# hammershock/SFM-Python

Hardware: AMD Instinct MI355X
Metric: BA iterations/sec (higher is better)
Workload: dtype f64

## Files before the change

### include/sfmba.h

```cpp
#ifndef SFMBA_H
#define SFMBA_H

#include <stdint.h>

#ifdef __cplusplus
extern "C" {
#endif

typedef struct sfmba_handle sfmba_handle;

typedef struct sfmba_options {
    double  ftol;
    double  xtol;
    double  gtol;
    int64_t max_nfev;
    int32_t verbose;
    int32_t max_iter;
    double  pcg_tol;
    int32_t pcg_max_iter;
    int32_t pcg_check_every;
    double  reg_min;
    int32_t profile;
    int32_t reserved;
    double  pcg_tol_max;
// ... 160 lines not shown
void sfmba_default_pose_options(sfmba_pose_options* opt);
int  sfmba_recover_pose(sfmba_handle* h, int64_t n_edges, const int64_t* edge_ptr, const double* pts1, const double* pts2,
                        const uint8_t* pair_use , const double* E, const double* K,
                        const sfmba_pose_options* opt, double* R, double* t, uint8_t* front_mask, double* X, double* angle_deg,
                        int32_t* edge_front, int32_t* edge_front_all, double* edge_sum_err, int32_t* edge_status,
                        int64_t* n_ok, double* kernel_us);

int  sfmba_set_descriptors(sfmba_handle* h, int64_t n_images, const int64_t* img_ptr ,
                           const void* desc , int32_t dtype ,
                           int32_t dim , int32_t* form_out);
typedef struct sfmba_match_options {
    double  ratio;
    int32_t form;
    int32_t profile;
} sfmba_match_options;
void sfmba_default_match_options(sfmba_match_options* opt);
int  sfmba_match_descriptors(sfmba_handle* h, int64_t n_edges, const int32_t* edges ,
                             const sfmba_match_options* opt, int64_t* query_ptr , int32_t* idx ,
                             double* dist_sq , uint8_t* good , int32_t* edge_good, int32_t* edge_status,
                             int64_t* n_ok, double* kernel_us);

int  sfmba_solve(sfmba_handle* h, double* x_inout, const sfmba_options* opt, sfmba_result* out);
int  sfmba_solve_from(sfmba_handle* h, const double* x0, double* x_out, const sfmba_options* opt, sfmba_result* out);
int  sfmba_get_fun_grad(sfmba_handle* h, double* fun_out, double* grad_out);

int  sfmba_time_kernel(sfmba_handle* h, const double* x, int32_t which, int32_t reps, double* avg_us);
int  sfmba_normal_blocks(sfmba_handle* h, const double* x, double* U, double* V, double* gc,
                         double* gp);
int  sfmba_schur_matvec(sfmba_handle* h, const double* x, const double* dc, const double* dp,
                        const double* v, double* y);

int  sfmba_step_products(sfmba_handle* h, const double* x, const double* sg, const double* dc, const double* dp_diag,
                         double* t1_out, double* g11_out, double* dp_out, double* sums_out, double* g_out, double* si_out);

int  sfmba_rhs_precond(sfmba_handle* h, const double* x, const double* dc, const double* dp, double* rhs_out,
                       double* sd_out, double* minv_out);

int  sfmba_dense_schur(sfmba_handle* h, const double* x, const double* dc, const double* dp, const double* rhs,
                       double* S_out, double* sol_out);

int  sfmba_tr2d_solve(const double* B3, const double* g2, double Delta, double* p2);
int  sfmba_debug_option(sfmba_handle* h, const char* name, int64_t value);

#ifdef __cplusplus
}
#endif
// ... 2 lines not shown
```

### sfm-python_amd/csrc/sfmba.hip

```cpp
#include "../../include/sfmba.h"

#include <hip/hip_runtime.h>
#include <hip/hip_ext.h>
#include <rccl/rccl.h>
#include <dlfcn.h>

#include <algorithm>
#include <atomic>
#include <chrono>
#include <cmath>
#include <cstdarg>
#include <cstdio>
#include <cstdlib>
#include <cstring>
#include <condition_variable>
#include <functional>
#include <initializer_list>
#include <mutex>
#include <numeric>
#include <string>
#include <thread>
#include <vector>

#include "problem_tables.hpp"
#include "ba_kernels.hpp"
#include "consumer_kernels.hpp"
#include "match_kernels.hpp"
#include "tr2d.hpp"

using namespace sfmba;

namespace {

constexpr size_t kLdsBytes = 160 * 1024;
constexpr size_t kLdsDynMax = kLdsBytes - 2048;
constexpr int kScalSlots = 32;
constexpr int kPartRows = 2048;
constexpr int kCostSlot = 0, kG11Slot = 1, kTailSlot = 2, kQ1Slot = 8;
constexpr int kMaxSlot = 12, kRegSlot = 13, kGhPrevSlot = 14, kEtaSlot = 15, kCamSlot = 16;
constexpr int kStepSlot = 25, kSkipSlot = 30, kRadiusSlot = 31;
constexpr int kPinCtrl = 40;
constexpr int kPinP2pErr = 62;
constexpr int kPointSlot[9] = {12, 8, 9, 10, 11, 4, 5, 6, 7};

struct DevBuf {
    void* p = nullptr;
    size_t bytes = 0;
// ... 23 lines not shown

struct DevView {
    void* p = nullptr;
    template <class T> T* as() const { return static_cast<T*>(p); }
};

struct PinnedBuf {
    void* p = nullptr;
    size_t bytes = 0;
    ~PinnedBuf() { if (p) (void)hipHostFree(p); }
    hipError_t ensure(size_t n, size_t keep) {
        if (n <= bytes && p) return hipSuccess;
        void* q = nullptr;
        const size_t cap = n + n / 2 + 64;
        hipError_t e = hipHostMalloc(&q, cap, hipHostMallocDefault);
        if (e != hipSuccess) return e;
        if (p && keep) memcpy(q, p, std::min(keep, bytes));
        if (p) (void)hipHostFree(p);
        p = q; bytes = cap;
        return hipSuccess;
    }
    template <class T> T* as() const { return static_cast<T*>(p); }
};

struct RcclApi {
    void* lib = nullptr;
    ncclResult_t (*GetUniqueId)(ncclUniqueId*) = nullptr;
    ncclResult_t (*CommInitRank)(ncclComm_t*, int, ncclUniqueId, int) = nullptr;
    ncclResult_t (*AllReduce)(const void*, void*, size_t, ncclDataType_t, ncclRedOp_t, ncclComm_t, hipStream_t) = nullptr;
    ncclResult_t (*CommDestroy)(ncclComm_t) = nullptr;
    const char* (*GetErrorString)(ncclResult_t) = nullptr;
};
RcclApi* rccl_api() {
    static RcclApi api;
    static bool tried = false;
    if (!tried) {
        tried = true;
        void* lib = dlopen("librccl.so.1", RTLD_NOW | RTLD_GLOBAL);
        if (!lib) lib = dlopen("librccl.so", RTLD_NOW | RTLD_GLOBAL);
        if (!lib) lib = dlopen("/opt/rocm/lib/librccl.so.1", RTLD_NOW | RTLD_GLOBAL);
        if (lib) {
            api.GetUniqueId = (decltype(api.GetUniqueId))dlsym(lib, "ncclGetUniqueId");
            api.CommInitRank = (decltype(api.CommInitRank))dlsym(lib, "ncclCommInitRank");
            api.AllReduce = (decltype(api.AllReduce))dlsym(lib, "ncclAllReduce");
            api.CommDestroy = (decltype(api.CommDestroy))dlsym(lib, "ncclCommDestroy");
            api.GetErrorString = (decltype(api.GetErrorString))dlsym(lib, "ncclGetErrorString");
// ... 8 lines not shown
    X(pcg_fused, -1)       \
    X(tab_lds, -1)         \
    X(vec_lds, -1)         \
    X(sweep_rc, -1)        \
    X(dense, -1)           \
    X(precond, -1)         \
    X(pcg_local, -1)       \
    X(xcd_chunks, -1)      \
    X(rhsrec, -1)          \
    X(cost_rider, -1)      \
    X(packed_upload, -1)   \
    X(jfree, -1)           \
    X(rc_consumers, -1)    \
    X(cm_device, -1)       \
    X(pcg_inline, -1)      \
    X(xcd_cam, -1)         \
    X(pcg_skip_last, -1)   \
    X(pcg_mixed_b, -1)     \
    X(pcg_mixed, -1)       \
    X(pcg_split, -1)       \
    X(spec_scale, -1)      \
    X(start_handoff, -1)   \
    X(early_download, -1)  \
    X(cam_chunk, 0)        \
    X(pcg_guess_bias, 0)   \
    X(trace_pcg, 0) X(trace_stalls, 0) X(trace_timing, 0)    \
    X(wait_deadline_s, 120)  \
    X(p2p_delay_ms, 0)     \
    X(p2p_timeout_ms, 0)
struct Debug {
#define X(name, init) int name = init;
    SFMBA_DEBUG_OPTIONS(X)
#undef X
};
const struct { const char* name; int Debug::*member; } kDebugOptions[] = {
#define X(name, init) {#name, &Debug::name},
    SFMBA_DEBUG_OPTIONS(X)
#undef X
};

struct Forms {
    bool packed_upload = false;
    bool cm_device = false;
    int64_t cam_chunk_len = 4096;
    bool lds_tab = true, lds_vec = true;
    bool sweep_rc = false;
// ... 93 lines not shown
        double* camdata[kP2pMaxRanks] = {};
        unsigned* words = nullptr;
        int64_t calls = 0;
        bool first_in_solve = true;
        int shared_device = 1;
        bool any_multi = false;
    } p2p;
    double* h_scal = nullptr;
    struct Stage { PinnedBuf uv, ci, pi, perm, ptr, uvf, tables, ci16, uv16; } stage;
    DevBuf ci16_dev, uv16_dev;
    struct Prev { bool valid = false; bool f32 = false; bool packed = false; int64_t N = 0, P = 0; } prev;
    ProblemTables tb;
    HostPool pool;
    int64_t obs_reused = 0, obs_uploaded = 0;
    double* mbox = nullptr;
    double* mbox_dev = nullptr;
    unsigned long long mbox_seq = 0;
    Mailbox post{};
    double* h_x = nullptr;
    size_t h_x_doubles = 0;
    hipStream_t copy_stream = nullptr;
    hipEvent_t ev_written = nullptr, ev_copied[2] = {nullptr, nullptr};
    bool result_in_flight = false;
    PinnedBuf mirror[2];
    unsigned long long mirror_tag[2] = {0, 0}, copy_count = 0, x_tag = 0;
    bool mirror_on = false;
    const double* skip = nullptr;
    double pcg_tol = 0.0; int pcg_cap = 0;
    bool pcg_b_owed = false;
    bool pcg_a_owed = false;
    DevBuf pcg_part;
    int pcg_hint = 0;
    std::vector<int> pcg_hist;
    int64_t hist_C = 0, hist_P = 0, hist_N = 0;
    unsigned long long hist_sig = 0;
    unsigned long long problem_gen = 0;
    bool solved = false;
    bool transport_dropped = false;
    std::vector<const void*> lds_ready;
    int last_pcg_iters = 0;

    double *x = nullptr, *x_new = nullptr;
    double *tab = nullptr, *tab_new = nullptr;
    double *rec = nullptr, *rec_new = nullptr;
    double *g_cur = nullptr, *si_cur = nullptr, *sg_cur = nullptr;
    double *g_new = nullptr, *si_new = nullptr, *sg_new = nullptr;
// ... 704 lines not shown
    CHK(exchange(h, h->scal() + kQ1Slot, 4, 0));
    CHK(exchange(h, h->scal() + kMaxSlot, 1, 1));
    return 0;
}

int fetch_scalars(sfmba_handle* h) {
    const Mailbox mb{h->mbox_dev, h->scal(), nullptr, ++h->mbox_seq, p2p_error_word(h)};
    hipLaunchKernelGGL(k_post, dim3(1), dim3(64), 0, h->stream, mb);
    LAUNCHED(h);
    CHK(wait_mailbox(h, h->mbox_seq));
    memcpy(h->h_scal, h->mbox, sizeof(double) * kScalSlots);
    return 0;
}

int ensure_h_x(sfmba_handle* h) {
    const size_t need = (size_t)std::max<int64_t>(h->n, 2 * h->N);
    if (h->h_x && h->h_x_doubles >= need) return 0;
    if (h->h_x) { (void)hipHostFree(h->h_x); h->h_x = nullptr; h->h_x_doubles = 0; }
    HIPCHK(h, hipHostMalloc((void**)&h->h_x, sizeof(double) * need, hipHostMallocDefault));
    h->h_x_doubles = need;
    return 0;
}

template <class Fn>
void staging_copy(sfmba_handle* h, void* dst, const void* src, size_t bytes, Fn chunk_done) {
    const int parts = (int)std::min<size_t>(4, bytes >> 19);
    if (parts <= 1) { memcpy(dst, src, bytes); chunk_done(0, (size_t)0, bytes); return; }
    const size_t per = ((bytes + parts - 1) / parts + 63) & ~(size_t)63;
    std::atomic<int> done[8];
    for (auto& d : done) d.store(0, std::memory_order_relaxed);
    h->pool.run(parts, [&](int t) {
        const size_t b = std::min(bytes, (size_t)t * per), e = std::min(bytes, b + per);
        if (e > b) memcpy(static_cast<char*>(dst) + b, static_cast<const char*>(src) + b, e - b);
        if (t != 0) { done[t].store(1, std::memory_order_release); return; }
        chunk_done(0, b, e - b);
        for (int k = 1; k < parts; ++k) {
            while (done[k].load(std::memory_order_acquire) == 0) { }
            const size_t bk = std::min(bytes, (size_t)k * per), ek = std::min(bytes, bk + per);
            chunk_done(k, bk, ek - bk);
        }
    });
}
void staging_copy(sfmba_handle* h, void* dst, const void* src, size_t bytes) {
    staging_copy(h, dst, src, bytes, [](int, size_t, size_t) {});
}

int upload_x(sfmba_handle* h, const double* x_host, double* dst = nullptr) {
    CHK(ensure_h_x(h));
    if (h->forms.mixed && !dst) {
        const double* pts = x_host + 6 * h->C;
        const int64_t stride = std::max<int64_t>(1, h->P / 1024);
        double sx = 0.0, sy = 0.0, sz = 0.0;
        int64_t cnt = 0;
        for (int64_t q = 0; q < h->P; q += stride, ++cnt) { sx += pts[3 * q]; sy += pts[3 * q + 1]; sz += pts[3 * q + 2]; }
        h->origin = Origin{sx / (double)cnt, sy / (double)cnt, sz / (double)cnt};
        if (!std::isfinite(h->origin.x + h->origin.y + h->origin.z)) h->origin = Origin{0.0, 0.0, 0.0};
    }
    HIPCHK(h, hipStreamSynchronize(h->stream));
    if (h->result_in_flight && h->copy_stream) HIPCHK(h, hipStreamSynchronize(h->copy_stream));
    h->result_in_flight = false;
    const double t0 = now_s();
    hipError_t err = hipSuccess;
    staging_copy(h, h->h_x, x_host, sizeof(double) * h->n, [&](int, size_t off, size_t bytes) {
        if (bytes == 0 || err != hipSuccess) return;
        err = hipMemcpyAsync(reinterpret_cast<char*>(dst ? dst : h->x) + off, reinterpret_cast<const char*>(h->h_x) + off, bytes,
                             hipMemcpyHostToDevice, h->stream);
    });
    HIPCHK(h, err);
    if (h->dbg.trace_timing) fprintf(stderr, "sfmba: upload_x  staging copy + enqueue %.1f us\n", 1e6 * (now_s() - t0));
    return 0;
}

int download_residuals(sfmba_handle* h, double* r_out) {
    CHK(ensure_h_x(h));
    HIPCHK(h, hipStreamSynchronize(h->stream));
    const size_t bytes = (h->f32 ? sizeof(float) : sizeof(double)) * 2 * (size_t)h->N;
    HIPCHK(h, hipMemcpyAsync(h->h_x, h->r.p, bytes, hipMemcpyDeviceToHost, h->stream));
    CHK(wait_stream(h));
    if (!h->f32 && !h->permuted) { memcpy(r_out, h->h_x, bytes); return 0; }
    const float* sf = reinterpret_cast<const float*>(h->h_x);
    for (int64_t k = 0; k < h->N; ++k) {
        const int64_t d = h->permuted ? h->tb.order[k] : k;
        r_out[2 * d] = h->f32 ? (double)sf[2 * k] : h->h_x[2 * k];
        r_out[2 * d + 1] = h->f32 ? (double)sf[2 * k + 1] : h->h_x[2 * k + 1];
    }
    return 0;
// ... 176 lines not shown
    o->reg_min = 1e-6; o->profile = 0; o->reserved = 0; o->pcg_tol_max = 0.1;
}

int sfmba_create(sfmba_handle** out, int device_id) {
    if (!out) return -1;
    *out = nullptr;
    int ndev = 0;
    hipError_t e = hipGetDeviceCount(&ndev);
    if (e != hipSuccess || ndev <= 0) return -3;
    if (device_id < 0 || device_id >= ndev) return -1;
    auto* h = new sfmba_handle();
    h->device = device_id;
    if (hipSetDevice(device_id) != hipSuccess) { delete h; return -3; }
    hipDeviceProp_t prop;
    if (hipGetDeviceProperties(&prop, device_id) == hipSuccess) h->n_cu = prop.multiProcessorCount;
    if (hipStreamCreateWithFlags(&h->stream, hipStreamNonBlocking) != hipSuccess) { delete h; return -3; }
    h->own_stream = true;
    if (hipHostMalloc((void**)&h->h_scal, sizeof(double) * 64, hipHostMallocDefault) != hipSuccess ||
        hipHostMalloc((void**)&h->mbox, sizeof(double) * 64, hipHostMallocCoherent | hipHostMallocMapped) != hipSuccess ||
        hipHostGetDevicePointer((void**)&h->mbox_dev, h->mbox, 0) != hipSuccess) {
        (void)hipStreamDestroy(h->stream); delete h; return -4;
    }
    memset(h->mbox, 0, sizeof(double) * 64);
    {
        int prio_low = 0, prio_high = 0;
        if (hipDeviceGetStreamPriorityRange(&prio_low, &prio_high) != hipSuccess) prio_low = 0;
        if (hipStreamCreateWithPriority(&h->copy_stream, hipStreamNonBlocking, prio_low) != hipSuccess) h->copy_stream = nullptr;
    }
    if (h->copy_stream &&
        (hipEventCreateWithFlags(&h->ev_written, hipEventDisableTiming) != hipSuccess ||
         hipEventCreateWithFlags(&h->ev_copied[0], hipEventDisableTiming) != hipSuccess ||
         hipEventCreateWithFlags(&h->ev_copied[1], hipEventDisableTiming) != hipSuccess)) {
        (void)hipStreamDestroy(h->copy_stream);
        h->copy_stream = nullptr;
    }
    *out = h;
    return 0;
}

void sfmba_destroy(sfmba_handle* h) {
    if (!h) return;
    (void)hipSetDevice(h->device);
    if (h->stream) (void)hipStreamSynchronize(h->stream);
    if (h->comm) { if (RcclApi* api = rccl_api()) (void)api->CommDestroy(h->comm); h->comm = nullptr; }
    p2p_release(h);
    if (h->copy_stream) { (void)hipStreamSynchronize(h->copy_stream); (void)hipStreamDestroy(h->copy_stream); }
    if (h->ev_written) (void)hipEventDestroy(h->ev_written);
    for (auto& ev : h->ev_copied) if (ev) (void)hipEventDestroy(ev);
    if (h->own_stream && h->stream) (void)hipStreamDestroy(h->stream);
    if (h->h_scal) (void)hipHostFree(h->h_scal);
    if (h->mbox) (void)hipHostFree(h->mbox);
    if (h->h_x) (void)hipHostFree(h->h_x);
    delete h;
}

const char* sfmba_last_error(const sfmba_handle* h) { return h ? h->err.c_str() : "null handle"; }

int sfmba_set_stream(sfmba_handle* h, void* hip_stream) {
    CHK(enter(h));
    if (h->stream) HIPCHK(h, hipStreamSynchronize(h->stream));
    if (h->own_stream && h->stream) (void)hipStreamDestroy(h->stream);
    h->stream = static_cast<hipStream_t>(hip_stream);
    h->own_stream = false;
    return 0;
}

int sfmba_set_print(sfmba_handle* h, sfmba_print_fn fn, void* ctx) {
    CHK(enter(h));
    h->print_fn = fn;
    h->print_ctx = ctx;
    return 0;
}

int sfmba_debug_option(sfmba_handle* h, const char* name, int64_t value) {
    CHK(enter(h));
// ... 1843 lines not shown
    struct EventList : std::vector<std::pair<hipEvent_t, hipEvent_t>> {
        ~EventList() { for (auto& pr : *this) { (void)hipEventDestroy(pr.first); (void)hipEventDestroy(pr.second); } }
    } evs;
    int np_cost = 0;
    int np_tail = 0;
    double cost = 0.0, Delta = -1.0;
    unsigned long long start_seq = 0;
    int64_t nfev = 1, njev = 1, iteration = 0, pcg_total = 0, pcg_breakdowns = 0;
    int status = -1;
    double step_norm = 0.0, actual_reduction = 0.0, g_norm = 0.0, reg_term = 0.0, cost_new = 0.0;
    bool have_red = false;
    int pcg_guess = h->pcg_hint;
    bool guess_exact = false;
    bool hist_same = false;
    unsigned long long sig = 0;
    std::vector<int> pcg_hist_new;
    int pcg_enqueued = 0;
    bool missed = false;
    PcgCtrl hc{};
    bool nb_valid = true;
    Mailbox trial_post{};
    bool trial_post_pending = false;
    bool result_sent = false;
    double t_begin = 0.0, t_dev0 = 0.0, t_sent0 = 0.0, t_sent1 = 0.0;

    int run(const double* x_start, double* x_out);
    int start(const double* x_start), start_values();
    void recall_pcg_record(const double* x_start);
    int linear_phase(), tail();
    int device_trial();
    void record_pcg_count();
    int step_loop(), accept_or_reject(), terminate();
    int deliver(double* x_out);
    int eval_jac(const double* x, double* tab, bool table_ready, bool finish = true);
    int enqueue_trial(const double* coef_dev, double c1, double c2), handoff(bool with_ctrl);
    int fetch() {
        CHK(wait_mailbox(h, h->mbox_seq));
        memcpy(h->h_scal, h->mbox, sizeof(double) * kScalSlots);
        return 0;
    }
    double qsum(int q) const { return hs[kPointSlot[q]] + hs[kCamSlot + q]; }
    int guess_launches() const { return pcg_guess + (f.pcg_fused ? 1 : 0) + (guess_exact ? 0 : 1); }
};

int Solve::eval_jac(const double* x, double* tab, bool table_ready, bool finish) {
    if (!table_ready) CHK(launch_cam_table(h, x, tab, h->rec, f.quick_start));
// ... 268 lines not shown
        if (term != 0) { status = term; break; }
        Delta = Delta_new;
    }
    have_red = true;
    return 0;
}

int Solve::accept_or_reject() {
    if (!(actual_reduction > 0.0)) {
        step_norm = 0.0;
        actual_reduction = 0.0;
        return 0;
    }
    std::swap(h->x, h->x_new);
    std::swap(h->tab, h->tab_new);
    std::swap(h->rec, h->rec_new);
    h->x_tag = h->mirror_tag[h->x == h->xa.as<double>() ? 0 : 1];
    nb_valid = true;
    cost = cost_new;
    ++njev;
    if (status != -1 && f.early_download && !h->mirror_on) {
        CHK(ensure_h_x(h));
        t_sent0 = now_s();
        HIPCHK(h, hipMemcpyAsync(h->h_x, h->x, sizeof(double) * (size_t)n, hipMemcpyDeviceToHost, h->copy_stream));
        HIPCHK(h, hipEventRecord(h->ev_copied[0], h->copy_stream));
        h->result_in_flight = true;
        result_sent = true;
        t_sent1 = now_s();
    }
    if (!f.spec_scale) return launch_update_scale(h, 0, true);
    std::swap(h->g_cur, h->g_new);
    std::swap(h->si_cur, h->si_new);
    std::swap(h->sg_cur, h->sg_new);
    h->pending_scale_sums = true;
    return 0;
}

int Solve::terminate() {
    if (h->pending_scale_sums) {
        CHK(flush_scale_sums(h));
        CHK(exchange_linearise(h));
    }
    CHK(fetch_scalars(h));
    g_norm = std::max(hs[kMaxSlot], hs[kCamSlot + 0]);
    if (opt.verbose >= 2) print_iter(h, iteration, nfev, cost, have_red, actual_reduction, step_norm, g_norm);
    return 0;
}

int Solve::deliver(double* x_out) {
    if (!nb_valid) {
        int np = 0;
        CHK((launch_resjac<false, true>(h, h->x, h->tab, &np)));
    }
    CHK(ensure_h_x(h));
    const double t_dl0 = now_s();
    const int xw = h->x == h->xa.as<double>() ? 0 : 1;
    const bool mirrored = h->mirror_on && h->x_tag != 0 && h->mirror_tag[xw] == h->x_tag;
    const size_t xbytes = sizeof(double) * (size_t)n;
    if (!mirrored && !result_sent) HIPCHK(h, hipMemcpyAsync(h->h_x, h->x, xbytes, hipMemcpyDeviceToHost, h->stream));
    if (h->p2p.ready)
        HIPCHK(h, hipMemcpyAsync(h->h_scal + kPinP2pErr, h->p2p.words + 1, sizeof(unsigned), hipMemcpyDeviceToHost, h->stream));
    CHK(wait_stream(h));
    const double t_ws = now_s();
    if (result_sent) {
        CHK(wait_stream(h, h->ev_copied[0]));
        h->result_in_flight = false;
    }
    if (mirrored) HIPCHK(h, hipEventSynchronize(h->ev_copied[xw]));
    const double t_dl1 = now_s();
    if (h->p2p.ready) {
        unsigned err = 0;
        memcpy(&err, h->h_scal + kPinP2pErr, sizeof err);
        if (err != 0) return p2p_timed_out(h, err);
    }
    staging_copy(h, x_out, mirrored ? h->mirror[xw].p : (const void*)h->h_x, xbytes);
    if (h->mirror_on) HIPCHK(h, hipStreamSynchronize(h->copy_stream));
    const double t_end = now_s();
    if (h->dbg.trace_timing && result_sent)
        fprintf(stderr, "sfmba: early result copy: enqueue %.1f us, then %.1f us to the last post, stream query %.1f us, copy event %.1f us\n",
                1e6 * (t_sent1 - t_sent0), 1e6 * (t_dl0 - t_sent1), 1e6 * (t_ws - t_dl0), 1e6 * (t_dl1 - t_ws));
    if (h->dbg.trace_timing)
        fprintf(stderr, "sfmba: solve  %.3f ms total, upload %.1f us, result: copy + wait %.1f us, staging copy %.1f us\n", 1e3 * (t_end - t_begin),
                1e6 * (t_dev0 - t_begin), 1e6 * (t_dl1 - t_dl0), 1e6 * (t_end - t_dl1));
    if (!evs.empty()) {
        double tot = 0.0;
        for (auto& pr : evs) {
            float ms = 0.f;
            if (hipEventElapsedTime(&ms, pr.first, pr.second) == hipSuccess) tot += ms;
        }
        out->resjac_avg_us = 1e3 * tot / (double)evs.size();
        out->resjac_launches = (int64_t)evs.size();
    }
    h->pcg_hist.swap(pcg_hist_new);
    h->hist_C = C; h->hist_P = P; h->hist_N = h->N; h->hist_sig = sig;
    out->cost = cost;
    out->optimality = g_norm;
    out->rmse = std::sqrt(2.0 * cost / m_total);
    out->nfev = nfev; out->njev = njev; out->iterations = iteration; out->pcg_iterations = pcg_total;
    out->status = status == -1 ? 0 : status;
    out->seconds_total = t_end - t_begin;
    out->seconds_device = t_end - t_dev0;
    out->last_step_norm = step_norm;
    out->last_reg = reg_term;
    out->reserved = (int32_t)pcg_breakdowns;
    h->solved = true;
    return 0;
}

int Solve::run(const double* x_start, double* x_out) {
    CHK(start(x_start));
    recall_pcg_record(x_start);
    if (opt.verbose >= 2) print_header(h);
    for (;;) {
        CHK(linear_phase());
        CHK(device_trial());
        g_norm = std::max(hs[kMaxSlot], hs[kCamSlot + 0]);
        if (g_norm < opt.gtol) status = 1;
        if (opt.verbose >= 2) print_iter(h, iteration, nfev, cost, have_red, actual_reduction, step_norm, g_norm);
        if (status != -1 || nfev >= max_nfev || (opt.max_iter > 0 && iteration >= opt.max_iter)) break;
        record_pcg_count();
        CHK(step_loop());
        CHK(accept_or_reject());
        ++iteration;
        if (status != -1) { CHK(terminate()); break; }
    }
    return deliver(x_out);
}

int solve_impl(sfmba_handle* h, const double* x_start, double* x_inout, const sfmba_options* opt_in, sfmba_result* out) {
    CHK(enter(h));
    CHK(begin_compute(h, x_start));
    if (!x_inout) return fail(h, -1, "x_out is NULL");
    if (!out) return fail(h, -1, "result is NULL");
    sfmba_options opt;
    if (opt_in) opt = *opt_in; else sfmba_default_options(&opt);
    memset(out, 0, sizeof *out);
    Solve s{h, opt, out};
    return s.run(x_start, x_inout);
}
}

int sfmba_solve(sfmba_handle* h, double* x_inout, const sfmba_options* opt_in, sfmba_result* out) {
    return sfmba_solve_from(h, x_inout, x_inout, opt_in, out);
}

int sfmba_solve_from(sfmba_handle* h, const double* x0, double* x_out, const sfmba_options* opt_in, sfmba_result* out) {
    const int rc = solve_impl(h, x0, x_out, opt_in, out);
    if (rc != 0 && h) {
        const std::string msg = h->err;
        h->skip = nullptr; h->post = Mailbox{};
        if (h->stream) (void)hipStreamSynchronize(h->stream);
        if (h->copy_stream) (void)hipStreamSynchronize(h->copy_stream);
        if (rc == -5 && h->p2p.ready) {
            p2p_close_peers(h);
            if (h->p2p.words) (void)hipMemset(h->p2p.words, 0, 4 * sizeof(unsigned));
        }
        h->err = msg;
    }
    return rc;
}

int sfmba_get_fun_grad(sfmba_handle* h, double* fun_out, double* grad_out) {
    CHK(enter(h));
    if (!h->have_problem || !h->solved) return fail(h, -1, "no completed sfmba_solve on this handle");
    if (fun_out) CHK(download_residuals(h, fun_out));
    if (grad_out) {
        CHK(ensure_h_x(h));
        HIPCHK(h, hipMemcpyAsync(h->h_x, h->g_cur, sizeof(double) * h->n, hipMemcpyDeviceToHost, h->stream));
        CHK(wait_stream(h));
// ... 11 lines not shown
```

### sfm-python_amd/sfmba/_capi.py

```python
from __future__ import annotations

import ctypes as C
import os

import numpy as np

_HERE = os.path.dirname(os.path.abspath(__file__))
LIB_PATH = os.environ.get("SFMBA_LIB") or os.path.join(_HERE, "libsfmba.so")

SYMBOLS = (
    "sfmba_create", "sfmba_destroy", "sfmba_last_error", "sfmba_default_options", "sfmba_set_stream",
    "sfmba_set_problem", "sfmba_set_problem_i64", "sfmba_exchange_doubles", "sfmba_set_exchange", "sfmba_residuals",
    "sfmba_residual_jacobian", "sfmba_solve", "sfmba_solve_from", "sfmba_get_fun_grad", "sfmba_time_kernel",
    "sfmba_normal_blocks", "sfmba_schur_matvec", "sfmba_comm_get_unique_id", "sfmba_comm_init",
    "sfmba_comm_destroy", "sfmba_set_precision", "sfmba_p2p_export", "sfmba_p2p_attach", "sfmba_p2p_detach",
    "sfmba_p2p_calls", "sfmba_tr2d_solve", "sfmba_debug_option", "sfmba_set_print", "sfmba_get_counters", "sfmba_problem_reuse", "sfmba_dense_schur",
    "sfmba_get_pcg_history", "sfmba_set_fixed_cameras", "sfmba_step_products", "sfmba_get_form", "sfmba_rhs_precond",
    "sfmba_default_filter_options", "sfmba_reprojection_stats",
    "sfmba_default_triangulate_options", "sfmba_triangulate",
    "sfmba_default_resect_options", "sfmba_resect",
    "sfmba_default_pnp_ransac_options", "sfmba_resect_ransac",
    "sfmba_default_ransac_options", "sfmba_fundamental_ransac", "sfmba_default_pose_options", "sfmba_recover_pose",
    "sfmba_set_descriptors", "sfmba_default_match_options", "sfmba_match_descriptors",
)


class Options(C.Structure):
    _fields_ = [("ftol", C.c_double), ("xtol", C.c_double), ("gtol", C.c_double),
                ("max_nfev", C.c_int64), ("verbose", C.c_int32), ("max_iter", C.c_int32),
                ("pcg_tol", C.c_double), ("pcg_max_iter", C.c_int32), ("pcg_check_every", C.c_int32),
                ("reg_min", C.c_double), ("profile", C.c_int32), ("reserved", C.c_int32),
                ("pcg_tol_max", C.c_double)]


class Result(C.Structure):
    _fields_ = [("cost", C.c_double), ("cost0", C.c_double), ("optimality", C.c_double),
                ("rmse", C.c_double), ("rmse0", C.c_double), ("nfev", C.c_int64), ("njev", C.c_int64),
                ("iterations", C.c_int64), ("pcg_iterations", C.c_int64), ("status", C.c_int32),
                ("reserved", C.c_int32), ("seconds_total", C.c_double), ("seconds_device", C.c_double),
                ("resjac_avg_us", C.c_double), ("resjac_launches", C.c_int64),
                ("last_step_norm", C.c_double), ("last_reg", C.c_double)]


class FilterOptions(C.Structure):
    _fields_ = [("max_error_px", C.c_double), ("min_depth", C.c_double), ("min_angle_deg", C.c_double),
                ("min_views", C.c_int32), ("reserved", C.c_int32)]
# ... 125 lines not shown
        lib.sfmba_default_pnp_ransac_options.restype = None
        lib.sfmba_resect_ransac.argtypes = ([P] * 5 + [C.POINTER(PnpRansacOptions)] + [P] * 12 +
                                            [C.POINTER(C.c_int64), C.POINTER(C.c_double)])
        lib.sfmba_resect_ransac.restype = C.c_int
    if hasattr(lib, "sfmba_fundamental_ransac"):
        lib.sfmba_default_ransac_options.argtypes = [C.POINTER(RansacOptions)]
        lib.sfmba_default_ransac_options.restype = None
        lib.sfmba_fundamental_ransac.argtypes = ([P, C.c_int64] + [P] * 5 + [C.POINTER(RansacOptions)] + [P] * 8 +
                                                 [C.POINTER(C.c_int64), C.POINTER(C.c_double)])
        lib.sfmba_fundamental_ransac.restype = C.c_int
        lib.sfmba_default_pose_options.argtypes = [C.POINTER(PoseOptions)]
        lib.sfmba_default_pose_options.restype = None
        lib.sfmba_recover_pose.argtypes = ([P, C.c_int64] + [P] * 6 + [C.POINTER(PoseOptions)] + [P] * 9 +
                                           [C.POINTER(C.c_int64), C.POINTER(C.c_double)])
        lib.sfmba_recover_pose.restype = C.c_int
    if hasattr(lib, "sfmba_match_descriptors"):
        lib.sfmba_set_descriptors.argtypes = [P, C.c_int64, P, P, C.c_int32, C.c_int32, C.POINTER(C.c_int32)]
        lib.sfmba_set_descriptors.restype = C.c_int
        lib.sfmba_default_match_options.argtypes = [C.POINTER(MatchOptions)]
        lib.sfmba_default_match_options.restype = None
        lib.sfmba_match_descriptors.argtypes = ([P, C.c_int64, P, C.POINTER(MatchOptions)] + [P] * 6 +
                                                [C.POINTER(C.c_int64), C.POINTER(C.c_double)])
        lib.sfmba_match_descriptors.restype = C.c_int
    lib.sfmba_tr2d_solve.argtypes = [P, P, C.c_double, P]
    lib.sfmba_comm_get_unique_id.argtypes = [P]
    lib.sfmba_comm_init.argtypes = [P, P, C.c_int32, C.c_int32, C.c_int64]
    lib.sfmba_comm_destroy.argtypes = [P]
    lib.sfmba_set_precision.argtypes = [P, C.c_int32]
    lib.sfmba_p2p_export.argtypes = [P, C.c_int32, P]
    lib.sfmba_p2p_attach.argtypes = [P, P, C.c_int32, C.c_int32]
    lib.sfmba_p2p_detach.argtypes = [P]
    lib.sfmba_debug_option.argtypes = [P, C.c_char_p, C.c_int64]
    lib.sfmba_problem_reuse.argtypes = [P, C.POINTER(C.c_int64), C.POINTER(C.c_int64)]
    lib.sfmba_problem_reuse.restype = C.c_int
    lib.sfmba_get_counters.argtypes = [P, C.POINTER(C.c_int64), C.POINTER(C.c_int64)]
    lib.sfmba_get_counters.restype = C.c_int
    lib.sfmba_get_pcg_history.argtypes = [P, P, C.c_int32]
    lib.sfmba_get_pcg_history.restype = C.c_int32
    lib.sfmba_set_print.argtypes = [P, PRINT_FN, P]
    lib.sfmba_set_print.restype = C.c_int
    lib.sfmba_set_fixed_cameras.argtypes = [P, P, C.c_int64]
    lib.sfmba_set_fixed_cameras.restype = C.c_int
    lib.sfmba_p2p_calls.argtypes = [P]
    lib.sfmba_p2p_calls.restype = C.c_int64
    for name in ("sfmba_set_stream", "sfmba_set_problem", "sfmba_set_problem_i64", "sfmba_set_exchange", "sfmba_residuals",
                 "sfmba_residual_jacobian", "sfmba_solve", "sfmba_solve_from", "sfmba_get_fun_grad", "sfmba_time_kernel",
# ... 11 lines not shown
```

### sfm-python_amd/sfmba/api.py

```python
from __future__ import annotations

import threading

import numpy as np

from . import _capi
from .backend import Backend

TERMINATION_MESSAGES = {
    -1: "Improper input parameters status returned from `leastsq`",
    0: "The maximum number of function evaluations is exceeded.",
    1: "`gtol` termination condition is satisfied.",
    2: "`ftol` termination condition is satisfied.",
    3: "`xtol` termination condition is satisfied.",
    4: "Both `ftol` and `xtol` termination conditions are satisfied.",
}

try:
    from scipy.optimize import OptimizeResult
except Exception:
    class OptimizeResult(dict):
        __getattr__ = dict.get
        __setattr__ = dict.__setitem__

# ... 362 lines not shown
        q[i] = 0.25 * s
        q[j] = (R[j, i] + R[i, j]) / s
        q[k] = (R[k, i] + R[i, k]) / s
        q[3] = (R[k, j] - R[j, k]) / s
    if q[3] < 0:
        q = -q
    nv = np.linalg.norm(q[:3])
    if nv < 1e-12:
        return 2.0 * q[:3]
    return q[:3] * (2.0 * np.arctan2(nv, q[3]) / nv)


def _matrix_from_rotvec(w):
    w = np.asarray(w, dtype=np.float64)
    th = np.linalg.norm(w)
    Wx = np.array([[0, -w[2], w[1]], [w[2], 0, -w[0]], [-w[1], w[0], 0]])
    if th < 1e-4:
        a, b = 1.0 - th * th / 6.0, 0.5 - th * th / 24.0
    else:
        a, b = np.sin(th) / th, 0.5 * (np.sin(0.5 * th) / (0.5 * th)) ** 2
    return np.eye(3) + a * Wx + b * (Wx @ Wx)


def pack_cameras_points(H_list, registered, X3d, observations, pose_convention="reference"):
    if pose_convention not in ("reference", "rt"):
        raise ValueError("pose_convention must be 'reference' or 'rt'")
    data = list(observations)
    pt_indices = np.array([d[0] for d in data])
    cam_ids = [d[1] for d in data]
    pt2ds = np.array([d[2] for d in data])
    reg = [k for k, f in enumerate(registered) if f]
    camera_map = {k: i for i, k in enumerate(reg)}
    params = []
    for k in reg:
        H = np.asarray(H_list[k], dtype=np.float64)
        T = H[:3, 3].flatten() if pose_convention == "reference" else -H[:3, :3].T @ H[:3, 3]
        params.append(np.hstack([_rotvec_from_matrix(H[:3, :3]), T]))
    camera_indices = np.array([camera_map[c] for c in cam_ids])
    X3d = np.asarray(X3d, dtype=np.float64)
    x0 = np.hstack([np.hstack(params).ravel(), X3d.ravel()])
    return x0, len(reg), len(X3d), camera_indices, pt_indices, pt2ds, camera_map


def unpack_cameras_points(x, n_cam, n_points, camera_map, H_list, pose_convention="reference"):
    cams = np.asarray(x[:n_cam * 6]).reshape((n_cam, 6))
    H_out = [np.array(H, dtype=np.float64, copy=True) for H in H_list]
    for cam_id, k in camera_map.items():
        H = np.eye(4)
        H[:3, :3] = _matrix_from_rotvec(cams[k, :3])
        H[:3, 3] = cams[k, 3:] if pose_convention == "reference" else -H[:3, :3] @ cams[k, 3:]
        H_out[cam_id] = H
    return H_out, np.asarray(x[n_cam * 6:]).reshape((n_points, 3))


def apply_bundle_adjustment(H_list, registered, X3d, observations, K, tol=1e-10, verbose=2, device=0,
                            pose_convention="reference"):
    x0, n_cam, n_points, ci, pi, uv, cmap = pack_cameras_points(H_list, registered, X3d, observations,
                                                                pose_convention)
    jac_sparsity = create_sparsity_matrix(n_cam, n_points, len(ci), ci, pi)
    res = least_squares(compute_residuals, x0, jac_sparsity=jac_sparsity, verbose=verbose, x_scale="jac",
                        ftol=tol, method="trf", args=(n_cam, n_points, ci, pi, uv, K), device=device)
    return unpack_cameras_points(res.x, n_cam, n_points, cmap, H_list, pose_convention) + (res,)
```

### sfm-python_amd/sfmba/backend.py

```python
from __future__ import annotations

import ctypes as C
import dataclasses

import weakref

import numpy as np

from . import _capi


class FundamentalEstimate:

    OK, FEW_PAIRS, DEGENERATE = 0, 1, 2

    def __init__(self, F, F_refit, inlier_mask, inliers, best, success, status, hyp_inliers, n_ok, kernel_us, edge_ptr):
        self.F, self.F_refit, self.inlier_mask = F, F_refit, inlier_mask
        self.inliers, self.best, self.success, self.status = inliers, best, success, status
        self.hyp_inliers, self.n_ok, self.kernel_us, self.edge_ptr = hyp_inliers, int(n_ok), float(kernel_us), edge_ptr

    @property
    def ok(self):
        return self.status == self.OK

# ... 204 lines not shown
    cameras: np.ndarray
    hyp: np.ndarray
    inlier_mask: np.ndarray
    status: np.ndarray
    views: np.ndarray
    inliers: np.ndarray
    best: np.ndarray
    best_sol: np.ndarray
    success: np.ndarray
    iters: np.ndarray
    rms_err: np.ndarray
    hyp_inliers: object
    n_ok: int
    kernel_us: float

    @property
    def ok(self):
        return self.status == self.OK

    def __repr__(self):
        return f"RobustResection(n_cameras={len(self.status)}, n_ok={self.n_ok})"


class Backend:

    def __init__(self, device: int = 0):
        self._lib = _capi.load()
        self._h = C.c_void_p()
        rc = self._lib.sfmba_create(C.byref(self._h), int(device))
        if rc != 0:
            self._h = None
            raise BackendError(
                f"sfmba_create(device={device}) failed with code {rc}: no usable MI355X/HIP device. "
                "The bundle-adjustment path has no CPU fallback.")
        self.device = int(device)
        self.n_cameras = self.n_points = self.n_obs = 0
        self._keep = []
        self._print_cb = _capi.PRINT_FN(lambda ctx, line: print(line.decode("utf-8", "replace")))
        self._lib.sfmba_set_print(self._h, self._print_cb, None)

    def close(self):
        if getattr(self, "_h", None):
            try:
                self._flush_pending()
            except Exception:
                pass
            self._lib.sfmba_destroy(self._h)
            self._h = None

    def __del__(self):
        try:
            self.close()
        except Exception:
            pass

    def _check(self, rc: int):
        if rc == 0:
            return
        msg = self._lib.sfmba_last_error(self._h).decode("utf-8", "replace")
        if rc in (-1, -2):
# ... 14 lines not shown

    def fetch_fun_grad(self, want_fun=True, want_grad=True):
        fun = np.empty(2 * self.n_obs) if want_fun else None
        grad = np.empty(self.n_params) if want_grad else None
        if want_fun or want_grad:
            self._check(self._lib.sfmba_get_fun_grad(self._h, _capi.ptr(fun) if want_fun else None,
                                                     _capi.ptr(grad) if want_grad else None))
        return fun, grad

    def set_precision(self, storage_bits: int):
        self._flush_pending()
        self._check(self._lib.sfmba_set_precision(self._h, int(storage_bits)))

    def set_fixed_cameras(self, camera_indices=()):
        idx = np.ascontiguousarray(sorted(set(int(c) for c in camera_indices)), dtype=np.int64)
        if tuple(idx) == getattr(self, "_fixed", ()):
            return
        self._flush_pending()
        self._check(self._lib.sfmba_set_fixed_cameras(self._h, _capi.ptr(idx) if len(idx) else None, len(idx)))
        self._fixed = tuple(int(c) for c in idx)

    def debug_option(self, name: str, value: int):
        self._check(self._lib.sfmba_debug_option(self._h, name.encode(), int(value)))

    def set_stream(self, hip_stream: int):
        self._check(self._lib.sfmba_set_stream(self._h, C.c_void_p(int(hip_stream))))

    def set_problem(self, n_cameras, n_points, camera_indices, point_indices, points_2d, K):
        self._flush_pending()
        ci = np.ascontiguousarray(camera_indices, dtype=np.int64).ravel()
        pi = np.ascontiguousarray(point_indices, dtype=np.int64).ravel()
        if ci.shape != pi.shape:
            raise ValueError("camera_indices and point_indices differ in length")
        n_obs = ci.shape[0]
        Kc = _f64(K, (3, 3), "K")
        p2 = np.asarray(points_2d)
        if p2.dtype == np.int64 and p2.shape == (n_obs, 2) and p2.flags.c_contiguous:
            self._check(self._lib.sfmba_set_problem_i64(self._h, int(n_cameras), int(n_points), n_obs,
                                                        _capi.ptr(ci), _capi.ptr(pi), _capi.ptr(p2),
                                                        _capi.ptr(Kc)))
        else:
            uv = _f64(points_2d, (n_obs, 2), "points_2d")
            self._check(self._lib.sfmba_set_problem(self._h, int(n_cameras), int(n_points), n_obs,
                                                    _capi.ptr(ci), _capi.ptr(pi), _capi.ptr(uv),
                                                    _capi.ptr(Kc)))
        self.n_cameras, self.n_points, self.n_obs = int(n_cameras), int(n_points), n_obs
# ... 351 lines not shown
        n = 6 * self.n_cameras
        S = np.empty((n, n))
        y = np.empty(n)
        self._check(self._lib.sfmba_dense_schur(self._h, _capi.ptr(x), _capi.ptr(dc), _capi.ptr(dp), _capi.ptr(rhs),
                                                _capi.ptr(S), _capi.ptr(y)))
        return S, y

    def time_kernel(self, x, which: int, reps: int) -> float:
        self._flush_pending()
        x = _f64(x, (self.n_params,), "x")
        us = C.c_double()
        self._check(self._lib.sfmba_time_kernel(self._h, _capi.ptr(x), int(which), int(reps),
                                                C.byref(us)))
        return us.value

    def default_options(self) -> _capi.Options:
        o = _capi.Options()
        self._lib.sfmba_default_options(C.byref(o))
        return o

    def solve(self, x0, options: _capi.Options | None = None, want_fun=True, want_grad=True):
        self._flush_pending()
        x_start = _f64(x0, (self.n_params,), "x0")
        x = np.empty_like(x_start)
        opt = options if options is not None else self.default_options()
        res = _capi.Result()
        self._check(self._lib.sfmba_solve_from(self._h, _capi.ptr(x_start), _capi.ptr(x), C.byref(opt), C.byref(res)))
        fun, grad = self.fetch_fun_grad(want_fun, want_grad)
        return x, res, fun, grad
```

Baseline: 2876.

## Allocate solve inputs and results in pooled pinned host blocks for direct DMA

Adds a refcounted pool of pinned host blocks exposed to Python. Solve results and packed initial parameters are placed in these blocks, so upload and download can DMA straight to and from user arrays. This skips the multi-threaded memcpy through the internal staging buffer. The cost is extra pinned allocations, a global mutex-protected map lookup on every solve, and lifetime handling of blocks through Python finalizers.

```diff
diff --git a/include/sfmba.h b/include/sfmba.h
--- a/include/sfmba.h
+++ b/include/sfmba.h
@@ -206,6 +206,9 @@
 
 int  sfmba_solve(sfmba_handle* h, double* x_inout, const sfmba_options* opt, sfmba_result* out);
 int  sfmba_solve_from(sfmba_handle* h, const double* x0, double* x_out, const sfmba_options* opt, sfmba_result* out);
+int  sfmba_result_alloc(sfmba_handle* h, int64_t n_doubles, double** out);
+int  sfmba_result_release(void* p);
+int  sfmba_result_pool_stats(sfmba_handle* h, int64_t* live, int64_t* cached, int64_t* bytes);
 int  sfmba_get_fun_grad(sfmba_handle* h, double* fun_out, double* grad_out);
 
 int  sfmba_time_kernel(sfmba_handle* h, const double* x, int32_t which, int32_t reps, double* avg_us);
diff --git a/sfm-python_amd/csrc/sfmba.hip b/sfm-python_amd/csrc/sfmba.hip
--- a/sfm-python_amd/csrc/sfmba.hip
+++ b/sfm-python_amd/csrc/sfmba.hip
@@ -23,6 +23,7 @@
 #include <vector>
 
 #include "problem_tables.hpp"
+#include "xfer.hpp"
 #include "ba_kernels.hpp"
 #include "consumer_kernels.hpp"
 #include "match_kernels.hpp"
@@ -92,6 +93,8 @@
     }
     template <class T> T* as() const { return static_cast<T*>(p); }
 };
+
+constexpr int kUploadParts = 4;
 
 struct RcclApi {
     void* lib = nullptr;
@@ -146,6 +149,8 @@
     X(spec_scale, -1)      \
     X(start_handoff, -1)   \
     X(early_download, -1)  \
+    X(result_pinned, -1)   \
+    X(max_parts, 0)        \
     X(cam_chunk, 0)        \
     X(pcg_guess_bias, 0)   \
     X(trace_pcg, 0) X(trace_stalls, 0) X(trace_timing, 0)    \
@@ -285,6 +290,8 @@
     hipStream_t copy_stream = nullptr;
     hipEvent_t ev_written = nullptr, ev_copied[2] = {nullptr, nullptr};
     bool result_in_flight = false;
+    BlockPool* blocks = nullptr;
+    int max_parts = kUploadParts;
     PinnedBuf mirror[2];
     unsigned long long mirror_tag[2] = {0, 0}, copy_count = 0, x_tag = 0;
     bool mirror_on = false;
@@ -1035,27 +1042,30 @@
     return 0;
 }
 
+constexpr int kResultParts = 4;
 template <class Fn>
-void staging_copy(sfmba_handle* h, void* dst, const void* src, size_t bytes, Fn chunk_done) {
-    const int parts = (int)std::min<size_t>(4, bytes >> 19);
-    if (parts <= 1) { memcpy(dst, src, bytes); chunk_done(0, (size_t)0, bytes); return; }
-    const size_t per = ((bytes + parts - 1) / parts + 63) & ~(size_t)63;
-    std::atomic<int> done[8];
+void staging_copy(sfmba_handle* h, void* dst, const void* src, size_t bytes, int max_parts, Fn chunk_done) {
+    const SlicePlan pl = slice_plan(bytes, max_parts);
+    if (pl.parts <= 1) { memcpy(dst, src, bytes); chunk_done(0, (size_t)0, bytes); return; }
+    std::atomic<int> done[kMaxSliceParts];
     for (auto& d : done) d.store(0, std::memory_order_relaxed);
-    h->pool.run(parts, [&](int t) {
-        const size_t b = std::min(bytes, (size_t)t * per), e = std::min(bytes, b + per);
+    h->pool.run(pl.parts, [&](int t) {
+        const size_t b = pl.begin(t), e = pl.end(t);
         if (e > b) memcpy(static_cast<char*>(dst) + b, static_cast<const char*>(src) + b, e - b);
         if (t != 0) { done[t].store(1, std::memory_order_release); return; }
         chunk_done(0, b, e - b);
-        for (int k = 1; k < parts; ++k) {
+        for (int k = 1; k < pl.parts; ++k) {
             while (done[k].load(std::memory_order_acquire) == 0) { }
-            const size_t bk = std::min(bytes, (size_t)k * per), ek = std::min(bytes, bk + per);
-            chunk_done(k, bk, ek - bk);
+            chunk_done(k, pl.begin(k), pl.end(k) - pl.begin(k));
         }
     });
 }
 void staging_copy(sfmba_handle* h, void* dst, const void* src, size_t bytes) {
-    staging_copy(h, dst, src, bytes, [](int, size_t, size_t) {});
+    staging_copy(h, dst, src, bytes, kResultParts, [](int, size_t, size_t) {});
+}
+
+bool in_pinned_block(const sfmba_handle* h, const void* p, size_t bytes) {
+    return h->blocks && h->dbg.result_pinned != 0 && p && h->blocks->owner_of(p, bytes) != nullptr;
 }
 
 int upload_x(sfmba_handle* h, const double* x_host, double* dst = nullptr) {
@@ -1073,8 +1083,14 @@
     if (h->result_in_flight && h->copy_stream) HIPCHK(h, hipStreamSynchronize(h->copy_stream));
     h->result_in_flight = false;
     const double t0 = now_s();
+    if (in_pinned_block(h, x_host, sizeof(double) * h->n)) {
+        HIPCHK(h, hipMemcpyAsync(dst ? dst : h->x, x_host, sizeof(double) * h->n, hipMemcpyHostToDevice, h->stream));
+        if (h->dbg.trace_timing) fprintf(stderr, "sfmba: upload_x  pinned source, enqueue %.1f us\n", 1e6 * (now_s() - t0));
+        return 0;
+    }
     hipError_t err = hipSuccess;
-    staging_copy(h, h->h_x, x_host, sizeof(double) * h->n, [&](int, size_t off, size_t bytes) {
+    const int parts = h->dbg.max_parts > 0 ? h->dbg.max_parts : h->max_parts;
+    staging_copy(h, h->h_x, x_host, sizeof(double) * h->n, parts, [&](int, size_t off, size_t bytes) {
         if (bytes == 0 || err != hipSuccess) return;
         err = hipMemcpyAsync(reinterpret_cast<char*>(dst ? dst : h->x) + off, reinterpret_cast<const char*>(h->h_x) + off, bytes,
                              hipMemcpyHostToDevice, h->stream);
@@ -1297,6 +1313,9 @@
         (void)hipStreamDestroy(h->stream); delete h; return -4;
     }
     memset(h->mbox, 0, sizeof(double) * 64);
+    h->blocks = new BlockPool(BlockAllocator{
+        [](size_t bytes, void*) -> void* { void* p = nullptr; return hipHostMalloc(&p, bytes, hipHostMallocDefault) == hipSuccess ? p : nullptr; },
+        [](void* p, void*) { (void)hipHostFree(p); }, nullptr});
     {
         int prio_low = 0, prio_high = 0;
         if (hipDeviceGetStreamPriorityRange(&prio_low, &prio_high) != hipSuccess) prio_low = 0;
@@ -1326,6 +1345,7 @@
     if (h->h_scal) (void)hipHostFree(h->h_scal);
     if (h->mbox) (void)hipHostFree(h->mbox);
     if (h->h_x) (void)hipHostFree(h->h_x);
+    delete h->blocks;
     delete h;
 }
 
@@ -3215,6 +3235,8 @@
     Mailbox trial_post{};
     bool trial_post_pending = false;
     bool result_sent = false;
+    double* landing = nullptr;
+    bool direct = false;
     double t_begin = 0.0, t_dev0 = 0.0, t_sent0 = 0.0, t_sent1 = 0.0;
 
     int run(const double* x_start, double* x_out);
@@ -3529,7 +3551,7 @@
     if (status != -1 && f.early_download && !h->mirror_on) {
         CHK(ensure_h_x(h));
         t_sent0 = now_s();
-        HIPCHK(h, hipMemcpyAsync(h->h_x, h->x, sizeof(double) * (size_t)n, hipMemcpyDeviceToHost, h->copy_stream));
+        HIPCHK(h, hipMemcpyAsync(landing, h->x, sizeof(double) * (size_t)n, hipMemcpyDeviceToHost, h->copy_stream));
         HIPCHK(h, hipEventRecord(h->ev_copied[0], h->copy_stream));
         h->result_in_flight = true;
         result_sent = true;
@@ -3564,7 +3586,7 @@
     const int xw = h->x == h->xa.as<double>() ? 0 : 1;
     const bool mirrored = h->mirror_on && h->x_tag != 0 && h->mirror_tag[xw] == h->x_tag;
     const size_t xbytes = sizeof(double) * (size_t)n;
-    if (!mirrored && !result_sent) HIPCHK(h, hipMemcpyAsync(h->h_x, h->x, xbytes, hipMemcpyDeviceToHost, h->stream));
+    if (!mirrored && !result_sent) HIPCHK(h, hipMemcpyAsync(landing, h->x, xbytes, hipMemcpyDeviceToHost, h->stream));
     if (h->p2p.ready)
         HIPCHK(h, hipMemcpyAsync(h->h_scal + kPinP2pErr, h->p2p.words + 1, sizeof(unsigned), hipMemcpyDeviceToHost, h->stream));
     CHK(wait_stream(h));
@@ -3580,7 +3602,7 @@
         memcpy(&err, h->h_scal + kPinP2pErr, sizeof err);
         if (err != 0) return p2p_timed_out(h, err);
     }
-    staging_copy(h, x_out, mirrored ? h->mirror[xw].p : (const void*)h->h_x, xbytes);
+    if (mirrored || !direct) staging_copy(h, x_out, mirrored ? h->mirror[xw].p : (const void*)h->h_x, xbytes);
     if (h->mirror_on) HIPCHK(h, hipStreamSynchronize(h->copy_stream));
     const double t_end = now_s();
     if (h->dbg.trace_timing && result_sent)
@@ -3615,7 +3637,10 @@
 }
 
 int Solve::run(const double* x_start, double* x_out) {
+    const uintptr_t a = (uintptr_t)x_start, b = (uintptr_t)x_out, len = sizeof(double) * (uintptr_t)n;
+    direct = in_pinned_block(h, x_out, len) && (a + len <= b || b + len <= a);
     CHK(start(x_start));
+    landing = direct ? x_out : h->h_x;
     recall_pcg_record(x_start);
     if (opt.verbose >= 2) print_header(h);
     for (;;) {
@@ -3651,7 +3676,35 @@
     return sfmba_solve_from(h, x_inout, x_inout, opt_in, out);
 }
 
+int sfmba_result_alloc(sfmba_handle* h, int64_t n_doubles, double** out) {
+    CHK(enter(h));
+    if (!out) return fail(h, -1, "out is NULL");
+    *out = nullptr;
+    if (n_doubles < 0) return fail(h, -1, "n_doubles is negative");
+    void* p = h->blocks->acquire(sizeof(double) * (size_t)n_doubles);
+    if (!p) return fail(h, -4, "sfmba_result_alloc: no pinned host memory for %lld doubles", (long long)n_doubles);
+    *out = static_cast<double*>(p);
+    return 0;
+}
+
+int sfmba_result_release(void* p) { return BlockPool::release(p) ? 0 : -1; }
+
+int sfmba_result_pool_stats(sfmba_handle* h, int64_t* live, int64_t* cached, int64_t* bytes) {
+    if (!h || !h->blocks) return -1;
+    h->blocks->stats(live, cached, bytes);
+    return 0;
+}
+
 int sfmba_solve_from(sfmba_handle* h, const double* x0, double* x_out, const sfmba_options* opt_in, sfmba_result* out) {
+    void* held[2] = {nullptr, nullptr};
+    if (h && h->blocks) {
+        const void* arrays[2] = {x0, x_out};
+        for (int k = 0; k < 2; ++k) {
+            void* b = arrays[k] ? h->blocks->owner_of(arrays[k], 1) : nullptr;
+            if (b && h->blocks->retain(b)) held[k] = b;
+        }
+    }
+    struct Unhold { void** held; ~Unhold() { for (int k = 0; k < 2; ++k) if (held[k]) (void)BlockPool::release(held[k]); } } unhold{held};
     const int rc = solve_impl(h, x0, x_out, opt_in, out);
     if (rc != 0 && h) {
         const std::string msg = h->err;
diff --git a/sfm-python_amd/csrc/xfer.hpp b/sfm-python_amd/csrc/xfer.hpp
--- /dev/null
+++ b/sfm-python_amd/csrc/xfer.hpp
@@ -0,0 +1,161 @@
+#pragma once
+
+#include <algorithm>
+#include <cstddef>
+#include <cstdint>
+#include <map>
+#include <mutex>
+#include <vector>
+
+namespace sfmba {
+
+constexpr int kMaxSliceParts = 8;
+struct SlicePlan {
+    int parts = 1;
+    size_t per = 0, bytes = 0;
+    size_t begin(int k) const { return std::min(bytes, (size_t)k * per); }
+    size_t end(int k) const { return std::min(bytes, begin(k) + per); }
+};
+inline SlicePlan slice_plan(size_t bytes, int max_parts) {
+    const int cap = std::max(1, std::min(max_parts, kMaxSliceParts));
+    const int parts = (int)std::min<size_t>((size_t)cap, bytes >> 19);
+    if (parts <= 1) return SlicePlan{1, bytes, bytes};
+    return SlicePlan{parts, ((bytes + (size_t)parts - 1) / (size_t)parts + 63) & ~(size_t)63, bytes};
+}
+
+struct BlockAllocator {
+    void* (*alloc)(size_t bytes, void* ctx) = nullptr;
+    void (*free)(void* p, void* ctx) = nullptr;
+    void* ctx = nullptr;
+};
+
+class BlockPool {
+public:
+    static constexpr int kMaxCached = 4;
+    static constexpr size_t kMinBlock = 4096;
+
+    explicit BlockPool(BlockAllocator a) : s_(new State) { s_->a = a; }
+    BlockPool(const BlockPool&) = delete;
+    BlockPool& operator=(const BlockPool&) = delete;
+    ~BlockPool() {
+        std::vector<void*> drop;
+        bool last;
+        const BlockAllocator a = s_->a;
+        {
+            std::lock_guard<std::mutex> lk(table().m);
+            s_->dead = true;
+            for (const Cached& c : s_->cached) drop.push_back(c.p);
+            s_->held -= cached_bytes(*s_);
+            s_->cached.clear();
+            last = s_->live == 0;
+        }
+        for (void* p : drop) a.free(p, a.ctx);
+        if (last) delete s_;
+    }
+
+    static size_t block_bytes(size_t bytes) {
+        size_t cap = kMinBlock;
+        while (cap < bytes) cap <<= 1;
+        return cap;
+    }
+
+    void* acquire(size_t bytes) {
+        if (bytes > ((size_t)1 << 46)) return nullptr;
+        const size_t cap = block_bytes(bytes);
+        {
+            std::lock_guard<std::mutex> lk(table().m);
+            for (size_t k = s_->cached.size(); k-- > 0;)
+                if (s_->cached[k].cap == cap) {
+                    void* p = s_->cached[k].p;
+                    s_->cached.erase(s_->cached.begin() + (ptrdiff_t)k);
+                    table().out[(uintptr_t)p] = Out{cap, 1, s_};
+                    ++s_->live;
+                    return p;
+                }
+        }
+        void* p = s_->a.alloc(cap, s_->a.ctx);
+        if (!p) return nullptr;
+        std::lock_guard<std::mutex> lk(table().m);
+        table().out[(uintptr_t)p] = Out{cap, 1, s_};
+        ++s_->live;
+        s_->held += (int64_t)cap;
+        return p;
+    }
+
+    bool retain(void* p) {
+        std::lock_guard<std::mutex> lk(table().m);
+        auto it = table().out.find((uintptr_t)p);
+        if (it == table().out.end() || it->second.pool != s_) return false;
+        ++it->second.refs;
+        return true;
+    }
+
+    static bool release(void* p) {
+        void* drop = nullptr;
+        State* gone = nullptr;
+        BlockAllocator a;
+        {
+            std::lock_guard<std::mutex> lk(table().m);
+            auto it = table().out.find((uintptr_t)p);
+            if (it == table().out.end()) return false;
+            if (--it->second.refs > 0) return true;
+            State* s = it->second.pool;
+            const size_t cap = it->second.cap;
+            table().out.erase(it);
+            --s->live;
+            a = s->a;
+            if (s->dead) {
+                drop = p;
+                s->held -= (int64_t)cap;
+                if (s->live == 0) gone = s;
+            } else {
+                s->cached.push_back(Cached{p, cap});
+                if ((int)s->cached.size() > kMaxCached) {
+                    drop = s->cached.front().p;
+                    s->held -= (int64_t)s->cached.front().cap;
+                    s->cached.erase(s->cached.begin());
+                }
+            }
+        }
+        if (drop) a.free(drop, a.ctx);
+        delete gone;
+        return true;
+    }
+
+    void* owner_of(const void* p, size_t bytes) const {
+        std::lock_guard<std::mutex> lk(table().m);
+        auto it = table().out.upper_bound((uintptr_t)p);
+        if (it == table().out.begin()) return nullptr;
+        --it;
+        const uintptr_t b = it->first, q = (uintptr_t)p;
+        if (it->second.pool != s_ || q >= b + it->second.cap || bytes > b + it->second.cap - q) return nullptr;
+        return (void*)b;
+    }
+
+    void stats(int64_t* live, int64_t* cached, int64_t* bytes) const {
+        std::lock_guard<std::mutex> lk(table().m);
+        if (live) *live = s_->live;
+        if (cached) *cached = (int64_t)s_->cached.size();
+        if (bytes) *bytes = s_->held;
+    }
+
+private:
+    struct Cached { void* p; size_t cap; };
+    struct State {
+        BlockAllocator a;
+        std::vector<Cached> cached;
+        int64_t live = 0, held = 0;
+        bool dead = false;
+    };
+    struct Out { size_t cap; int64_t refs; State* pool; };
+    struct Table { std::mutex m; std::map<uintptr_t, Out> out; };
+    static Table& table() { static Table* t = new Table; return *t; }
+    static int64_t cached_bytes(const State& s) {
+        int64_t b = 0;
+        for (const Cached& c : s.cached) b += (int64_t)c.cap;
+        return b;
+    }
+    State* s_;
+};
+
+}
diff --git a/sfm-python_amd/sfmba/_capi.py b/sfm-python_amd/sfmba/_capi.py
--- a/sfm-python_amd/sfmba/_capi.py
+++ b/sfm-python_amd/sfmba/_capi.py
@@ -22,6 +22,7 @@
     "sfmba_default_pnp_ransac_options", "sfmba_resect_ransac",
     "sfmba_default_ransac_options", "sfmba_fundamental_ransac", "sfmba_default_pose_options", "sfmba_recover_pose",
     "sfmba_set_descriptors", "sfmba_default_match_options", "sfmba_match_descriptors",
+    "sfmba_result_alloc", "sfmba_result_release", "sfmba_result_pool_stats",
 )
 
 
@@ -193,6 +194,13 @@
         lib.sfmba_match_descriptors.argtypes = ([P, C.c_int64, P, C.POINTER(MatchOptions)] + [P] * 6 +
                                                 [C.POINTER(C.c_int64), C.POINTER(C.c_double)])
         lib.sfmba_match_descriptors.restype = C.c_int
+    if hasattr(lib, "sfmba_result_alloc"):
+        lib.sfmba_result_alloc.argtypes = [P, C.c_int64, C.POINTER(P)]
+        lib.sfmba_result_alloc.restype = C.c_int
+        lib.sfmba_result_release.argtypes = [P]
+        lib.sfmba_result_release.restype = C.c_int
+        lib.sfmba_result_pool_stats.argtypes = [P] + [C.POINTER(C.c_int64)] * 3
+        lib.sfmba_result_pool_stats.restype = C.c_int
     lib.sfmba_tr2d_solve.argtypes = [P, P, C.c_double, P]
     lib.sfmba_comm_get_unique_id.argtypes = [P]
     lib.sfmba_comm_init.argtypes = [P, P, C.c_int32, C.c_int32, C.c_int64]
diff --git a/sfm-python_amd/sfmba/api.py b/sfm-python_amd/sfmba/api.py
--- a/sfm-python_amd/sfmba/api.py
+++ b/sfm-python_amd/sfmba/api.py
@@ -408,7 +408,7 @@
     return np.eye(3) + a * Wx + b * (Wx @ Wx)
 
 
-def pack_cameras_points(H_list, registered, X3d, observations, pose_convention="reference"):
+def pack_cameras_points(H_list, registered, X3d, observations, pose_convention="reference", backend=None):
     if pose_convention not in ("reference", "rt"):
         raise ValueError("pose_convention must be 'reference' or 'rt'")
     data = list(observations)
@@ -424,7 +424,11 @@
         params.append(np.hstack([_rotvec_from_matrix(H[:3, :3]), T]))
     camera_indices = np.array([camera_map[c] for c in cam_ids])
     X3d = np.asarray(X3d, dtype=np.float64)
-    x0 = np.hstack([np.hstack(params).ravel(), X3d.ravel()])
+    parts = [np.hstack(params).ravel(), X3d.ravel()]
+    if backend is None:
+        backend = next(iter((getattr(_local, "cache", None) or {}).values()), None)
+    x0 = backend.pinned_empty(sum(len(p) for p in parts)) if backend is not None else None
+    x0 = np.concatenate(parts, out=x0) if x0 is not None else np.hstack(parts)
     return x0, len(reg), len(X3d), camera_indices, pt_indices, pt2ds, camera_map
 
 
@@ -442,7 +446,7 @@
 def apply_bundle_adjustment(H_list, registered, X3d, observations, K, tol=1e-10, verbose=2, device=0,
                             pose_convention="reference"):
     x0, n_cam, n_points, ci, pi, uv, cmap = pack_cameras_points(H_list, registered, X3d, observations,
-                                                                pose_convention)
+                                                                pose_convention, backend=get_backend(device))
     jac_sparsity = create_sparsity_matrix(n_cam, n_points, len(ci), ci, pi)
     res = least_squares(compute_residuals, x0, jac_sparsity=jac_sparsity, verbose=verbose, x_scale="jac",
                         ftol=tol, method="trf", args=(n_cam, n_points, ci, pi, uv, K), device=device)
diff --git a/sfm-python_amd/sfmba/backend.py b/sfm-python_amd/sfmba/backend.py
--- a/sfm-python_amd/sfmba/backend.py
+++ b/sfm-python_amd/sfmba/backend.py
@@ -250,6 +250,18 @@
         return f"RobustResection(n_cameras={len(self.status)}, n_ok={self.n_ok})"
 
 
+class _PinnedBlock:
+
+    def __init__(self, release, address, n):
+        self._release, self._address = release, address
+        self.__array_interface__ = {"version": 3, "shape": (int(n),), "typestr": "<f8", "data": (address, False)}
+
+    def __del__(self):
+        release, self._release = self._release, None
+        if release is not None:
+            release(self._address)
+
+
 class Backend:
 
     def __init__(self, device: int = 0):
@@ -264,6 +276,7 @@
         self.device = int(device)
         self.n_cameras = self.n_points = self.n_obs = 0
         self._keep = []
+        self._pinned = hasattr(self._lib, "sfmba_result_alloc")
         self._print_cb = _capi.PRINT_FN(lambda ctx, line: print(line.decode("utf-8", "replace")))
         self._lib.sfmba_set_print(self._h, self._print_cb, None)
 
@@ -324,6 +337,21 @@
 
     def debug_option(self, name: str, value: int):
         self._check(self._lib.sfmba_debug_option(self._h, name.encode(), int(value)))
+        if name == "result_pinned":
+            self._pinned = int(value) != 0 and hasattr(self._lib, "sfmba_result_alloc")
+
+    def pinned_empty(self, n):
+        if not self._pinned or not self._h:
+            return None
+        p = C.c_void_p()
+        if self._lib.sfmba_result_alloc(self._h, int(n), C.byref(p)) != 0 or not p.value:
+            return None
+        return np.asarray(_PinnedBlock(self._lib.sfmba_result_release, p.value, n))
+
+    def result_pool_stats(self):
+        live, cached, nbytes = C.c_int64(), C.c_int64(), C.c_int64()
+        self._check(self._lib.sfmba_result_pool_stats(self._h, C.byref(live), C.byref(cached), C.byref(nbytes)))
+        return int(live.value), int(cached.value), int(nbytes.value)
 
     def set_stream(self, hip_stream: int):
         self._check(self._lib.sfmba_set_stream(self._h, C.c_void_p(int(hip_stream))))
@@ -721,7 +749,9 @@
     def solve(self, x0, options: _capi.Options | None = None, want_fun=True, want_grad=True):
         self._flush_pending()
         x_start = _f64(x0, (self.n_params,), "x0")
-        x = np.empty_like(x_start)
+        x = self.pinned_empty(x_start.shape[0])
+        if x is None:
+            x = np.empty_like(x_start)
         opt = options if options is not None else self.default_options()
         res = _capi.Result()
         self._check(self._lib.sfmba_solve_from(self._h, _capi.ptr(x_start), _capi.ptr(x), C.byref(opt), C.byref(res)))
```

Measured after the change: 2842. 1.2% lower.
